# axruff/cuda-flow2d

Hardware: AMD Instinct MI355X
Metric: Mpixels*SOR-iters/sec at finest level (whole-pyramid wall time); full-pyramid pairs/sec in pairs_per_s (higher is better)
Workload: dtype f32; 1 GPU; cfg3_4096_gradient; width=4096, height=4096, pyramid_levels=8, data_constancy=gradient, median_radius=5, relaxation=Jacobi, reference iteration counts (bit-exact parity mode), parallelism=independent pairs, one process per GPU, no data-path collective, streams_per_gpu=4, hip_graph_replay=True, steps_per_lock_step_group=8

## Files before the change

cuda-flow2d_amd/__init__.py:

```python
import ctypes as C
import math
import os
import subprocess

import numpy as np

_HERE = os.path.dirname(os.path.abspath(__file__))
ROOT = os.path.dirname(_HERE)
HIP_LIB_PATH = os.environ.get("FLOW2D_HIP_LIB") or os.path.join(_HERE, "csrc", "libflow2d_hip.so")
HOST_LIB_PATH = os.path.join(_HERE, "host", "libflow2d_host.so")
CLI_PATH = os.path.join(_HERE, "host", "flow2d")

GREY, GRADIENT, GRADIENT_UNTILED, LOG_DERIVATIVES = 0, 1, 2, 3
_HOST_CONSTANCY = {GREY: 0, GRADIENT: 1, GRADIENT_UNTILED: 3, LOG_DERIVATIVES: 2}
SOLVER_AUTO, SOLVER_PER_SWEEP, SOLVER_FUSED, SOLVER_SINGLE_WORKGROUP, SOLVER_TILED = 0, 1, 2, 3, 4
TRACK_ALIVE, TRACK_INACTIVE, TRACK_MOTION_BOUNDARY, TRACK_LEFT_FRAME, TRACK_OCCLUDED = 0, 1, 2, 3, 4
DEFAULT_MIN_EIGENVALUE = 1.0
MOTION_TRANSLATION, MOTION_SIMILARITY, MOTION_AFFINE = 0, 1, 2
MOTION_MODELS = {"translation": MOTION_TRANSLATION, "similarity": MOTION_SIMILARITY, "affine": MOTION_AFFINE}

STATUS = {0: "ok", 1: "invalid argument", 2: "no usable HIP device", 3: "HIP runtime error",
          4: "out of device memory", 5: "unsupported parameter"}


# ... 181 lines not shown
        L.flow2d_context_destroy.argtypes = [vp]
        L.flow2d_context_device.argtypes = [vp, C.POINTER(i)]
        L.flow2d_context_stream.argtypes = [vp, C.POINTER(vp)]
        L.flow2d_synchronize.argtypes = [vp]
        L.flow2d_context_set_batch.argtypes = [vp, sz, sz]
        L.flow2d_mem_info.argtypes = [vp, C.POINTER(sz), C.POINTER(sz)]
        L.flow2d_device_name.argtypes = [vp, C.c_char_p, sz]
        L.flow2d_plane_pitch_bytes.restype = sz
        L.flow2d_plane_pitch_bytes.argtypes = [sz]
        L.flow2d_plane_alloc.argtypes = [vp, sz, sz, C.POINTER(vp), C.POINTER(sz)]
        L.flow2d_plane_free.argtypes = [vp, vp]
        L.flow2d_memset_2d.argtypes = [vp, vp, sz, i, sz, sz]
        L.flow2d_copy_h2d_2d.argtypes = [vp, vp, sz, vp, sz, sz, sz]
        L.flow2d_copy_d2h_2d.argtypes = [vp, vp, sz, vp, sz, sz, sz]
        L.flow2d_copy_d2d.argtypes = [vp, vp, vp, sz]
        L.flow2d_copy_planes.argtypes = [vp, sz, C.POINTER(vp), C.POINTER(vp), sz, sz, sz]
        L.flow2d_event_create.argtypes = [vp, C.POINTER(vp)]
        L.flow2d_event_record.argtypes = [vp, vp]
        L.flow2d_event_synchronize.argtypes = [vp, vp]
        L.flow2d_event_elapsed_ms.argtypes = [vp, vp, vp, C.POINTER(f)]
        L.flow2d_event_destroy.argtypes = [vp, vp]
        L.flow2d_stream_wait_event.argtypes = [vp, vp]
        L.flow2d_host_alloc.argtypes = [vp, sz, C.POINTER(vp)]
        L.flow2d_host_free.argtypes = [vp, vp]
        L.flow2d_add_2d.argtypes = [vp, vp, vp, sz, sz, sz]
        L.flow2d_gaussian_kernel.argtypes = [f, C.POINTER(f), C.POINTER(i)]
        L.flow2d_convolution_rows.argtypes = [vp, vp, vp, sz, sz, sz, C.POINTER(f), i]
        L.flow2d_convolution_columns.argtypes = [vp, vp, vp, sz, sz, sz, C.POINTER(f), i]
        L.flow2d_gaussian_blur.argtypes = [vp, vp, vp, sz, sz, sz, C.POINTER(f), i]
        L.flow2d_median_2d.argtypes = [vp, vp, sz, sz, sz, sz, vp]
        L.flow2d_registration_2d.argtypes = [vp, vp, vp, vp, vp, sz, sz, sz, f, f, vp]
        L.flow2d_upsample_registration_2d.argtypes = [vp, vp, vp, sz, sz, vp, vp, vp, vp, sz, sz, sz, f, f, vp]
        L.flow2d_resample_x.argtypes = [vp, vp, vp, sz, sz, sz, sz]
        L.flow2d_resample_y.argtypes = [vp, vp, vp, sz, sz, sz, sz]
        L.flow2d_add_2d_pair.argtypes = [vp, vp, vp, vp, vp, sz, sz, sz]
        L.flow2d_median_2d_pair.argtypes = [vp, vp, vp, sz, sz, sz, sz, vp, vp]
        L.flow2d_add_median_2d_pair.argtypes = [vp, vp, vp, vp, vp, sz, sz, sz, sz, vp, vp]
        L.flow2d_resample_x_pair.argtypes = [vp, vp, vp, vp, vp, sz, sz, sz, sz]
        L.flow2d_resample_y_pair.argtypes = [vp, vp, vp, vp, vp, sz, sz, sz, sz]
        L.flow2d_resample_xy_pair.argtypes = [vp, vp, vp, vp, vp, sz, sz, sz, sz, sz]
        L.flow2d_resample_x_levels.argtypes = [vp, vp, vp, vp, vp, sz, sz, sz, sz, C.POINTER(sz), C.POINTER(sz)]
        L.flow2d_compute_phi_ksi.argtypes = [vp] * 7 + [sz, sz, sz, f, f, f, f, vp, vp]
        L.flow2d_solve_2d.argtypes = [vp] * 9 + [sz, sz, sz, f, f, f, vp, vp]
        L.flow2d_solve_2d_grad.argtypes = [vp] * 9 + [sz, sz, sz, f, f, f, vp, vp]
        L.flow2d_solve_2d_grad_untiled.argtypes = [vp] * 9 + [sz, sz, sz, f, f, f, vp, vp]
        L.flow2d_solve_2d_log.argtypes = [vp] * 9 + [sz, sz, sz, f, f, f, vp, vp]
        L.flow2d_solver_algorithm_for.argtypes = [i, sz, sz, sz, sz, sz, i]
        L.flow2d_solve_2d_sor.argtypes = [vp] * 9 + [sz, sz, sz, f, f, f, f, i]
        L.flow2d_solve_level.argtypes = [vp] * 11 + [C.POINTER(SolveParams), C.POINTER(i)]
        L.flow2d_timing_enable.argtypes = [vp, i]
        L.flow2d_fused_fallbacks.argtypes = [vp, C.POINTER(C.c_ulonglong)]
        L.flow2d_context_set_lone.argtypes = [vp, i]
        L.flow2d_resample_y_levels.argtypes = [vp, vp, vp, vp, vp, sz, sz, sz, C.POINTER(sz), C.POINTER(sz), C.POINTER(sz), C.POINTER(sz)]
        L.flow2d_clock_probe_start.argtypes = [vp, C.c_double]
        L.flow2d_clock_probe_read.argtypes = [vp, C.POINTER(C.c_double)]
        L.flow2d_fused_block_order.argtypes = [vp, sz, sz, sz, sz, C.POINTER(i), sz, C.POINTER(sz)]
        if hasattr(L, "flow2d_fused_plain_waves"):
            L.flow2d_fused_plain_waves.argtypes = [vp, C.POINTER(C.c_ulonglong)]
        L.flow2d_timing_launch_filter.argtypes = [vp, sz, sz]
        if hasattr(L, "flow2d_consistency_2d"):
            L.flow2d_consistency_2d.argtypes = [vp, vp, vp, vp, vp, sz, sz, sz, f, f, vp]
        if hasattr(L, "flow2d_interpolate_2d"):
            L.flow2d_interpolate_2d.argtypes = [vp] * 9 + [sz, sz, sz, f, i, f, vp]
        if hasattr(L, "flow2d_track_points_2d"):
            L.flow2d_track_points_2d.argtypes = [vp] * 5 + [sz, sz, sz, vp, vp, vp, sz, f, f, i, f, f, vp, vp, vp]
            L.flow2d_seed_points_workspace_bytes.restype = sz
            L.flow2d_seed_points_workspace_bytes.argtypes = [sz, sz, sz]
            L.flow2d_seed_points_2d.argtypes = [vp, vp, sz, sz, sz, sz, f, vp, vp, vp, sz, vp, vp, sz]
        if hasattr(L, "flow2d_denoise_2d"):
            L.flow2d_denoise_2d.argtypes = [vp, vp, sz, C.POINTER(vp), C.POINTER(vp), C.POINTER(vp), C.POINTER(vp), sz, sz, sz, f,
                                            vp, vp]
            L.flow2d_compose_flow_2d.argtypes = [vp] * 7 + [sz, sz, sz, vp, vp, vp]
        if hasattr(L, "flow2d_global_motion_2d"):
            d = C.c_double
            L.flow2d_global_motion_workspace_bytes.restype = sz
            L.flow2d_global_motion_workspace_bytes.argtypes = [sz, sz, sz]
            L.flow2d_global_motion_2d.argtypes = [vp, vp, vp, vp, sz, sz, sz, i, d, i, vp, vp, sz]
            L.flow2d_global_flow_2d.argtypes = [vp, vp, vp, vp, vp, sz, sz, sz, d, vp, vp, vp, vp, vp]
            L.flow2d_warp_global_2d.argtypes = [vp, vp, vp, sz, sz, sz, f, vp, vp]
        if hasattr(L, "flow2d_deformation_2d"):
            L.flow2d_deformation_workspace_bytes.restype = sz
            L.flow2d_deformation_workspace_bytes.argtypes = [sz, sz, sz]
            L.flow2d_deformation_2d.argtypes = [vp, vp, vp, vp, sz, sz, sz, i, C.POINTER(DeformationPlanes), vp, vp, sz]
        if hasattr(L, "flow2d_segment_motion_2d"):
            L.flow2d_segment_motion_workspace_bytes.restype = sz
            L.flow2d_segment_motion_workspace_bytes.argtypes = [sz, sz, sz]
            L.flow2d_segment_motion_2d.argtypes = [vp, vp, vp, vp, sz, sz, sz, f, f, C.c_uint, vp, vp, sz, vp, vp, sz]
        if hasattr(L, "flow2d_flow_error_2d"):
            L.flow2d_flow_error_workspace_bytes.restype = sz
            L.flow2d_flow_error_workspace_bytes.argtypes = [sz, sz, sz]
            L.flow2d_flow_error_2d.argtypes = [vp] * 6 + [sz, sz, sz, vp, vp, vp, vp, sz]
        L.flow2d_timing_count.argtypes = [vp, C.POINTER(sz)]
        L.flow2d_timing_get.argtypes = [vp, sz, C.POINTER(TimingRecord)]
        L.flow2d_timing_reset.argtypes = [vp]
        _hip = L
    return _hip


def _check(status, where):
    if status != 0:
        raise Flow2DError(status, where, hip_lib().flow2d_last_error().decode(errors="replace"))


def device_count():
    n = C.c_int(0)
    st = hip_lib().flow2d_device_count(C.byref(n))
    return n.value if st == 0 else 0


def gaussian_kernel(sigma):
    taps = (C.c_float * 51)()
    r = C.c_int(0)
    _check(hip_lib().flow2d_gaussian_kernel(sigma, taps, C.byref(r)), "flow2d_gaussian_kernel")
    return np.array(taps[: 2 * r.value + 1], np.float32), r.value


class Plane:

    def __init__(self, ctx, width, height):
        self.ctx = ctx
        self.width, self.height = width, height
        ptr, pitch = C.c_void_p(), C.c_size_t()
        _check(hip_lib().flow2d_plane_alloc(ctx.handle, width, height, C.byref(ptr), C.byref(pitch)),
               "flow2d_plane_alloc")
        self.ptr, self.pitch = ptr.value, pitch.value

    def upload(self, array):
        a = np.ascontiguousarray(array, np.float32)
        h, w = a.shape
        assert w <= self.width and h <= self.height
        _check(hip_lib().flow2d_copy_h2d_2d(self.ctx.handle, self.ptr, self.pitch, a.ctypes.data, w * 4, w * 4, h),
               "flow2d_copy_h2d_2d")
        self.ctx.synchronize()
        return self

    def download(self, width=None, height=None):
        w = self.width if width is None else width
        h = self.height if height is None else height
        out = np.empty((h, w), np.float32)
        _check(hip_lib().flow2d_copy_d2h_2d(self.ctx.handle, out.ctypes.data, w * 4, self.ptr, self.pitch, w * 4, h),
               "flow2d_copy_d2h_2d")
        self.ctx.synchronize()
        return out

    def fill_bytes(self, value=0):
        _check(hip_lib().flow2d_memset_2d(self.ctx.handle, self.ptr, self.pitch, value, self.width * 4, self.height),
               "flow2d_memset_2d")
        return self

    def free(self):
        if self.ptr:
            hip_lib().flow2d_plane_free(self.ctx.handle, self.ptr)
            self.ptr = None


class _BatchScope:
# ... 9 lines not shown


class Context:

    def __init__(self, device=0, stream=None):
        h = C.c_void_p()
        if stream is None:
            _check(hip_lib().flow2d_context_create(device, C.byref(h)), "flow2d_context_create")
        else:
            _check(hip_lib().flow2d_context_create_on_stream(device, stream, C.byref(h)),
                   "flow2d_context_create_on_stream")
        self.handle = h
        self._planes = []

    def plane(self, width, height, data=None):
        p = Plane(self, width, height)
        self._planes.append(p)
        if data is not None:
            p.fill_bytes(0)
            p.upload(data)
        return p

    def copy_planes(self, srcs, dsts, width, height):
        n = len(srcs)
        a, b = (C.c_void_p * n)(*[p.ptr for p in srcs]), (C.c_void_p * n)(*[p.ptr for p in dsts])
        _check(hip_lib().flow2d_copy_planes(self.handle, n, a, b, srcs[0].pitch, width, height), "flow2d_copy_planes")

    def synchronize(self):
        _check(hip_lib().flow2d_synchronize(self.handle), "flow2d_synchronize")

    def mem_info(self):
        a, b = C.c_size_t(), C.c_size_t()
        _check(hip_lib().flow2d_mem_info(self.handle, C.byref(a), C.byref(b)), "flow2d_mem_info")
        return a.value, b.value

    def fused_fallbacks(self):
        n = C.c_ulonglong()
        _check(hip_lib().flow2d_fused_fallbacks(self.handle, C.byref(n)), "flow2d_fused_fallbacks")
        return n.value

    def set_lone(self, lone):
        _check(hip_lib().flow2d_context_set_lone(self.handle, int(bool(lone))), "flow2d_context_set_lone")

    def set_batch(self, count, stride_bytes=0):
        _check(hip_lib().flow2d_context_set_batch(self.handle, count, stride_bytes), "flow2d_context_set_batch")
        return _BatchScope(self)

    def resample_y_levels(self, packed_a, out_a, in_height, widths, heights, columns, rows, packed_b=None, out_b=None):
        n = len(widths)
        arr = lambda v: (C.c_size_t * n)(*v)
        _check(hip_lib().flow2d_resample_y_levels(self.handle, packed_a.ptr, out_a.ptr, packed_b.ptr if packed_b else None,
                                                  out_b.ptr if out_b else None, in_height, packed_a.pitch, n, arr(widths), arr(heights),
                                                  arr(columns), arr(rows)), "flow2d_resample_y_levels")

    def clock_probe_start(self, duration_us):
        _check(hip_lib().flow2d_clock_probe_start(self.handle, float(duration_us)), "flow2d_clock_probe_start")

    def clock_probe_read(self):
        ghz = (C.c_double * 8)()
        _check(hip_lib().flow2d_clock_probe_read(self.handle, ghz), "flow2d_clock_probe_read")
        return list(ghz)

    def fused_block_order(self, width, height, inner, instances=1):
        grid = C.c_size_t(0)
        cap = 1 << 16
        buf = (C.c_int * (4 * cap))()
        _check(hip_lib().flow2d_fused_block_order(self.handle, width, height, inner, instances, buf, cap, C.byref(grid)),
               "flow2d_fused_block_order")
        return np.frombuffer(buf, np.int32, 4 * grid.value).reshape(-1, 4).copy()

    def fused_plain_waves(self):
        n = C.c_ulonglong()
        _check(hip_lib().flow2d_fused_plain_waves(self.handle, C.byref(n)), "flow2d_fused_plain_waves")
        return n.value

    def device_name(self):
        buf = C.create_string_buffer(256)
        _check(hip_lib().flow2d_device_name(self.handle, buf, 256), "flow2d_device_name")
        return buf.value.decode()

    def close(self):
        if self.handle:
            for p in self._planes:
                p.free()
            self._planes = []
            hip_lib().flow2d_context_destroy(self.handle)
            self.handle = None

    def __enter__(self):
        return self

    def __exit__(self, *exc):
        self.close()

    def event(self):
        e = C.c_void_p()
        _check(hip_lib().flow2d_event_create(self.handle, C.byref(e)), "flow2d_event_create")
        return e

    def record(self, ev):
        _check(hip_lib().flow2d_event_record(self.handle, ev), "flow2d_event_record")

    def wait_event(self, ev):
        _check(hip_lib().flow2d_event_synchronize(self.handle, ev), "flow2d_event_synchronize")

    def elapsed_ms(self, start, stop):
# ... 967 lines not shown
```

cuda-flow2d_amd/csrc/pyramid_ops.hip:

```cpp
#include <algorithm>
#include <cmath>
#include <type_traits>
#include <utility>

#include "common.hpp"

namespace {

constexpr int kBlockX = 64;
constexpr int kBlockY = 4;

inline dim3 grid_for(size_t w, size_t h) { return dim3(flow2d::div_up(w, kBlockX), flow2d::div_up(h, kBlockY)); }

__global__ __launch_bounds__(256) void add_2d_kernel(float* __restrict__ op0_a, const float* __restrict__ op1_a,
                                                     float* __restrict__ op0_b, const float* __restrict__ op1_b, int w,
                                                     int h, int pitch, BatchArg batch)
{
    float* __restrict__ op0 = (batch_plane(batch) ? op0_b : op0_a) + batch_offset(batch);
    const float* __restrict__ op1 = (batch_plane(batch) ? op1_b : op1_a) + batch_offset(batch);
    const int x4 = (blockIdx.x * kBlockX + threadIdx.x) * 4;
    const int y = blockIdx.y * kBlockY + threadIdx.y;
    if (y >= h || x4 >= w) return;
    const size_t off = static_cast<size_t>(y) * pitch + x4;
    if (x4 + 3 < w) {
        float4 a = *reinterpret_cast<const float4*>(op0 + off);
        const float4 b = *reinterpret_cast<const float4*>(op1 + off);
        a.x += b.x;
        a.y += b.y;
        a.z += b.z;
        a.w += b.w;
        *reinterpret_cast<float4*>(op0 + off) = a;
    } else {
        for (int i = 0; x4 + i < w; ++i) op0[off + i] += op1[off + i];
    }
}

struct GaussTaps {
    float t[51];
};

template <bool kRows>
__global__ __launch_bounds__(256) void gauss_kernel(float* __restrict__ dst, const float* __restrict__ src, int w,
                                                    int h, int pitch, int radius, GaussTaps taps)
{
    const int x = blockIdx.x * kBlockX + threadIdx.x;
    const int y = blockIdx.y * kBlockY + threadIdx.y;
    if (x >= w || y >= h) return;
    float sum = 0.f;
    for (int j = -radius; j <= radius; ++j) {
        float s;
        if (kRows) {
            const int xx = x + j;
            s = (xx >= 0 && xx < w) ? src[static_cast<size_t>(y) * pitch + xx] : 0.f;
// ... 709 lines not shown
    const int out_w = lv.out_w[l], out_h = lv.out_h[l], rows_per_thread = lv.rows_per_thread[l];
    const float delta = lv.delta[l], normalization = lv.normalization[l];
    const float* __restrict__ in = (batch_plane(batch) ? in_b : in_a) + batch_offset(batch) + lv.col[l];
    float* __restrict__ out = (batch_plane(batch) ? out_b : out_a) + batch_offset(batch) + static_cast<size_t>(lv.out_row[l]) * pitch;
    const int block = static_cast<int>(blockIdx.x) - lv.first_block[l], blocks_x = lv.blocks_x[l];
    const int block_y = block / blocks_x;
    const int x = (block - block_y * blocks_x) * kBlockX + threadIdx.x;
    if (x >= out_w) return;
    const float* base = in + x;
    const int max_cells = lv.max_cells[l];
    if (rows_per_thread == 4 && max_cells <= 2) return resample_y_rows<2, 4>(base, out, x, block_y, out_h, in_h, pitch, delta, normalization);
    if (rows_per_thread == 4 && max_cells <= 4) return resample_y_rows<4, 4>(base, out, x, block_y, out_h, in_h, pitch, delta, normalization);
    if (rows_per_thread == 4 && max_cells <= 9) return resample_y_rows<9, 4>(base, out, x, block_y, out_h, in_h, pitch, delta, normalization);
    if (rows_per_thread == 1 && max_cells <= 9) return resample_y_rows<9, 1>(base, out, x, block_y, out_h, in_h, pitch, delta, normalization);
    for (int row = 0; row < rows_per_thread; ++row) {
        const int y = (block_y * rows_per_thread + row) * kBlockY + threadIdx.y;
        if (y >= out_h) return;
        const float left_f = static_cast<float>(static_cast<unsigned>(y)) * delta;
        const float right_f = static_cast<float>(static_cast<unsigned>(y) + 1u) * delta;
        const int left_i = static_cast<int>(floorf(left_f));
        const int right_i = min(in_h, static_cast<int>(ceilf(right_f)));
        const int cells = right_i - left_i;
        const size_t stride = pitch;
        float value = 0.f;
        if (cells == 1) {
            value += base[static_cast<size_t>(left_i) * stride] * delta;
        } else if (cells > 1) {
            const int last = left_i + cells - 1;
            value += base[static_cast<size_t>(left_i) * stride] * (static_cast<float>(left_i + 1) - left_f);
            int k = left_i + 1;
            for (; k + 32 <= last; k += 32) {
                float v[32];
#pragma unroll
                for (int i = 0; i < 32; ++i) v[i] = base[static_cast<size_t>(k + i) * stride];
#pragma unroll
                for (int i = 0; i < 32; ++i) value += v[i];
            }
            for (; k < last; k += 8) {
                float v[8];
#pragma unroll
                for (int i = 0; i < 8; ++i) v[i] = base[static_cast<size_t>(min(k + i, last - 1)) * stride];
#pragma unroll
                for (int i = 0; i < 8; ++i) {
                    const float next = value + v[i];
                    value = k + i < last ? next : value;
                }
            }
            value += base[static_cast<size_t>(last) * stride] * (right_f - static_cast<float>(last));
        }
        out[static_cast<size_t>(y) * pitch + x] = value * normalization;
    }
}

}

extern "C" {

static int launch_add(flow2d_context* ctx, float* operand_0, const float* operand_1, float* operand_0_b,
                      const float* operand_1_b, size_t width, size_t height, size_t pitch_bytes)
{
    FLOW2D_ENTER(ctx);
    if (!flow2d::plane_args_ok(operand_0, width, height, pitch_bytes) ||
        !flow2d::plane_args_ok(operand_1, width, height, pitch_bytes))
        return FLOW2D_ERR_INVALID_ARGUMENT;
    const bool pair = operand_0_b || operand_1_b;
    if (pair && (!flow2d::plane_args_ok(operand_0_b, width, height, pitch_bytes) ||
                 !flow2d::plane_args_ok(operand_1_b, width, height, pitch_bytes) || operand_0_b == operand_0 ||
                 operand_0_b == operand_1 || operand_0 == operand_1_b))
        return FLOW2D_ERR_INVALID_ARGUMENT;
    const unsigned planes = pair ? 2 : 1;
    dim3 grid(flow2d::div_up(width, kBlockX * 4), flow2d::div_up(height, kBlockY), flow2d::batch_z(ctx, planes));
    add_2d_kernel<<<grid, dim3(kBlockX, kBlockY), 0, ctx->stream>>>(operand_0, operand_1, operand_0_b, operand_1_b,
                                                                   (int)width, (int)height, (int)(pitch_bytes / 4),
                                                                   flow2d::batch_arg(ctx, planes));
    FLOW2D_CHECK_LAUNCH();
    return FLOW2D_OK;
}

int flow2d_add_2d(flow2d_context* ctx, float* operand_0, const float* operand_1, size_t width, size_t height,
                  size_t pitch_bytes)
{
    return launch_add(ctx, operand_0, operand_1, nullptr, nullptr, width, height, pitch_bytes);
}

int flow2d_add_2d_pair(flow2d_context* ctx, float* operand_0_a, const float* operand_1_a, float* operand_0_b,
                       const float* operand_1_b, size_t width, size_t height, size_t pitch_bytes)
{
    if (!operand_0_b || !operand_1_b) return FLOW2D_ERR_INVALID_ARGUMENT;
    return launch_add(ctx, operand_0_a, operand_1_a, operand_0_b, operand_1_b, width, height, pitch_bytes);
}

namespace {
struct PlaneTable {
    const float* src[FLOW2D_COPY_PLANES_MAX];
    float* dst[FLOW2D_COPY_PLANES_MAX];
};
__global__ __launch_bounds__(256) void copy_planes_kernel(PlaneTable t, int width, int height, int pitch_floats)
{
    const float* src = t.src[blockIdx.z];
    float* dst = t.dst[blockIdx.z];
    const int quads = width >> 2;
    for (int y = blockIdx.y; y < height; y += gridDim.y) {
        const size_t row = static_cast<size_t>(y) * pitch_floats;
        for (int q = blockIdx.x * blockDim.x + threadIdx.x; q < quads; q += gridDim.x * blockDim.x)
            reinterpret_cast<float4*>(dst + row)[q] = reinterpret_cast<const float4*>(src + row)[q];
        const int x = (quads << 2) + blockIdx.x * blockDim.x + threadIdx.x;
// ... 198 lines not shown
        }
    }
    const size_t lds_bytes = (in_width + in_width / 32 + 1) * sizeof(float);
    resample_x_levels_kernel<<<dim3(static_cast<unsigned>(height), 1, flow2d::batch_z(ctx, planes)), 256, lds_bytes,
                               ctx->stream>>>(input_a, packed_a, input_b, packed_b, static_cast<int>(in_width),
                                              static_cast<int>(pitch), lv, flow2d::batch_arg(ctx, planes));
    FLOW2D_CHECK_LAUNCH();
    return FLOW2D_OK;
}

int flow2d_resample_y_levels(flow2d_context* ctx, const float* packed_a, float* output_a, const float* packed_b, float* output_b,
                             size_t in_height, size_t pitch_bytes, size_t level_count, const size_t* out_widths,
                             const size_t* out_heights, const size_t* column_offsets, const size_t* output_rows)
{
    FLOW2D_ENTER(ctx);
    if (!out_widths || !out_heights || !column_offsets || !output_rows || level_count == 0 || !packed_a || !output_a ||
        packed_a == output_a || pitch_bytes == 0 || pitch_bytes % 16 != 0 || in_height == 0)
        return FLOW2D_ERR_INVALID_ARGUMENT;
    if (level_count > FLOW2D_RESAMPLE_MAX_LEVELS) return FLOW2D_ERR_UNSUPPORTED;
    const bool pair = packed_b || output_b;
    if (pair && (!packed_b || !output_b || packed_b == output_b || output_b == output_a || output_b == packed_a || output_a == packed_b))
        return FLOW2D_ERR_INVALID_ARGUMENT;
    const size_t pitch = pitch_bytes / 4;
    ResampleYLevels lv{};
    lv.count = static_cast<int>(level_count);
    long blocks = 0;
    for (size_t l = 0; l <= FLOW2D_RESAMPLE_MAX_LEVELS; ++l) lv.first_block[l] = 0x7fffffff;
    for (size_t l = 0; l < level_count; ++l) {
        if (out_widths[l] == 0 || out_heights[l] == 0 || out_heights[l] >= (1u << 30) || column_offsets[l] + out_widths[l] > pitch ||
            output_rows[l] >= (1u << 30))
            return FLOW2D_ERR_INVALID_ARGUMENT;
        for (size_t m = 0; m < l; ++m)
            if (output_rows[l] < output_rows[m] + out_heights[m] && output_rows[m] < output_rows[l] + out_heights[l])
                return FLOW2D_ERR_INVALID_ARGUMENT;
        lv.out_w[l] = static_cast<int>(out_widths[l]), lv.out_h[l] = static_cast<int>(out_heights[l]);
        lv.col[l] = static_cast<int>(column_offsets[l]), lv.out_row[l] = static_cast<int>(output_rows[l]);
        const float out_n = static_cast<float>(out_heights[l]), in_n = static_cast<float>(in_height);
        lv.delta[l] = in_n / out_n, lv.normalization[l] = out_n / in_n;
        lv.rows_per_thread[l] = out_widths[l] * out_heights[l] >= (size_t)512 * 512 ? 4 : 1;
        lv.max_cells[l] = lv.delta[l] == std::floor(lv.delta[l]) && lv.delta[l] < 1e6f ? static_cast<int>(lv.delta[l])
                                                                                      : static_cast<int>(std::min(std::ceil(lv.delta[l]) + 2.f, 1e9f));
        lv.first_block[l] = static_cast<int>(blocks);
        lv.blocks_x[l] = static_cast<int>(flow2d::div_up(out_widths[l], kBlockX));
        blocks += static_cast<long>(lv.blocks_x[l]) * static_cast<long>(flow2d::div_up(flow2d::div_up(out_heights[l], lv.rows_per_thread[l]), kBlockY));
        if (blocks >= 0x7fffffffl) return FLOW2D_ERR_UNSUPPORTED;
    }
    const unsigned planes = pair ? 2 : 1;
    resample_y_levels_kernel<<<dim3(static_cast<unsigned>(blocks), 1, flow2d::batch_z(ctx, planes)), dim3(kBlockX, kBlockY), 0, ctx->stream>>>(
        packed_a, output_a, packed_b, output_b, static_cast<int>(in_height), static_cast<int>(pitch), lv, flow2d::batch_arg(ctx, planes));
    FLOW2D_CHECK_LAUNCH();
    return FLOW2D_OK;
}

int flow2d_resample_x(flow2d_context* ctx, const float* input, float* output, size_t out_width, size_t out_height,
                      size_t in_width, size_t pitch_bytes)
{
    return launch_resample(ctx, true, input, output, nullptr, nullptr, out_width, out_height, in_width, pitch_bytes);
}

int flow2d_resample_x_pair(flow2d_context* ctx, const float* input_a, float* output_a, const float* input_b,
                           float* output_b, size_t out_width, size_t out_height, size_t in_width, size_t pitch_bytes)
{
    if (!input_b || !output_b) return FLOW2D_ERR_INVALID_ARGUMENT;
    return launch_resample(ctx, true, input_a, output_a, input_b, output_b, out_width, out_height, in_width, pitch_bytes);
}

int flow2d_resample_y(flow2d_context* ctx, const float* input, float* output, size_t out_width, size_t out_height,
                      size_t in_height, size_t pitch_bytes)
{
    return launch_resample(ctx, false, input, output, nullptr, nullptr, out_width, out_height, in_height, pitch_bytes);
}

int flow2d_resample_y_pair(flow2d_context* ctx, const float* input_a, float* output_a, const float* input_b,
                           float* output_b, size_t out_width, size_t out_height, size_t in_height, size_t pitch_bytes)
{
    if (!input_b || !output_b) return FLOW2D_ERR_INVALID_ARGUMENT;
    return launch_resample(ctx, false, input_a, output_a, input_b, output_b, out_width, out_height, in_height,
                           pitch_bytes);
}

int flow2d_resample_xy_pair(flow2d_context* ctx, const float* input_a, float* output_a, const float* input_b,
                            float* output_b, size_t in_width, size_t in_height, size_t out_width, size_t out_height,
                            size_t pitch_bytes)
{
    FLOW2D_ENTER(ctx);
    if (!flow2d::plane_args_ok(input_a, in_width, in_height, pitch_bytes) ||
        !flow2d::plane_args_ok(output_a, out_width, out_height, pitch_bytes) || input_a == output_a)
        return FLOW2D_ERR_INVALID_ARGUMENT;
    const bool pair = input_b || output_b;
    if (pair && (!flow2d::plane_args_ok(input_b, in_width, in_height, pitch_bytes) ||
                 !flow2d::plane_args_ok(output_b, out_width, out_height, pitch_bytes) || input_b == output_b ||
                 output_b == output_a || output_b == input_a || output_a == input_b))
        return FLOW2D_ERR_INVALID_ARGUMENT;
    const unsigned planes = pair ? 2 : 1;
    dim3 grid = grid_for(out_width, flow2d::div_up(out_height, kResampleXYRows));
    grid.z = flow2d::batch_z(ctx, planes);
    const ResampleXY k{static_cast<float>(in_width) / static_cast<float>(out_width),
                       static_cast<float>(out_width) / static_cast<float>(in_width),
                       static_cast<float>(in_height) / static_cast<float>(out_height),
                       static_cast<float>(out_height) / static_cast<float>(in_height)};
    resample_xy_kernel<<<grid, dim3(kBlockX, kBlockY), 0, ctx->stream>>>(
        input_a, output_a, input_b, output_b, (int)out_width, (int)out_height, (int)in_width, (int)in_height,
        (int)(pitch_bytes / 4), k, flow2d::batch_arg(ctx, planes));
    FLOW2D_CHECK_LAUNCH();
    return FLOW2D_OK;
}
// ... 66 lines not shown
```

cuda-flow2d_amd/host/optical_flow_2d.cpp:

```cpp
#include "optical_flow_2d.h"

#include <algorithm>
#include <cmath>
#include <cstdio>

#include "host_entry.h"

size_t OpticalFlowBase2D::GetMaxWarpLevel(size_t width, size_t height, float scale_factor) const
{
    size_t level_w = 1, level_h = 1, levels = 1;
    for (; scale_factor < 1.f; ++levels) {
        const float s = std::pow(scale_factor, static_cast<float>(levels));
        level_w = static_cast<size_t>(std::ceil(width * s));
        level_h = static_cast<size_t>(std::ceil(height * s));
        if (level_w < 4 || level_h < 4) break;
    }
    if (level_w == 1 || level_h == 1) --levels;
    return levels;
}

bool OpticalFlowBase2D::IsInitialized() const
{
    if (!initialized_) std::printf("Error: '%s' was not initialized.\n", name_);
    return initialized_;
// ... 677 lines not shown
        DevicePtr temp = Acquire();
        for (int i = 0; i < 2; ++i) {
            FramePyramid& pyramid = *sequence_frames_[i];
            if (gaussian_sigma > 0.0) {
                pyramid.level0 = pyramid.blurred;
                if (!pyramid.valid) {
                    op.Clear();
                    op.PushValuePtr("dev_input", &callers[i]);
                    op.PushValuePtr("dev_output", &pyramid.level0);
                    op.PushValuePtr("dev_temp", &temp);
                    op.PushValuePtr("data_size", &original_size);
                    op.PushValuePtr("gaussian_sigma", &gaussian_sigma);
                    cuop_convolution_.Execute(op);
                failed |= cuop_convolution_.TakeFailure();
                }
            } else {
                pyramid.level0 = callers[i];
            }
            *level0[i] = pyramid.level0;
        }
        Release(temp);
    } else if (gaussian_sigma > 0.0 && caller_frame_0_) {
        DevicePtr temp = Acquire();
        DevicePtr sources[2] = {caller_frame_0_, caller_frame_1_};
        DevicePtr* targets[2] = {&frame_0, &frame_1};
        for (int i = 0; i < 2; ++i) {
            op.Clear();
            op.PushValuePtr("dev_input", &sources[i]);
            op.PushValuePtr("dev_output", targets[i]);
            op.PushValuePtr("dev_temp", &temp);
            op.PushValuePtr("data_size", &original_size);
            op.PushValuePtr("gaussian_sigma", &gaussian_sigma);
            cuop_convolution_.Execute(op);
            failed |= cuop_convolution_.TakeFailure();
        }
        Release(temp);
    } else if (gaussian_sigma > 0.0) {
        DevicePtr temp = Acquire();
        DevicePtr* io[2][2] = {{&frame_0, &flow_u}, {&frame_1, &flow_v}};
        for (auto& pair : io) {
            op.Clear();
            op.PushValuePtr("dev_input", pair[0]);
            op.PushValuePtr("dev_output", pair[1]);
            op.PushValuePtr("dev_temp", &temp);
            op.PushValuePtr("data_size", &original_size);
            op.PushValuePtr("gaussian_sigma", &gaussian_sigma);
            cuop_convolution_.Execute(op);
            failed |= cuop_convolution_.TakeFailure();
            std::swap(*pair[0], *pair[1]);
        }
        Release(temp);
    }

    if (packed) {
        if (CheckFlow2DError(flow2d_resample_x_levels(context_, AsPlane(frame_0), AsPlane(packed_frames_[0]),
                                                      AsPlane(frame_1), AsPlane(packed_frames_[1]),
                                                      original_size.width, original_size.height,
                                                      dev_container_size_.pitch, packed_width.size(),
                                                      packed_width.data(), packed_column.data()),
                             "flow2d_resample_x_levels"))
            failed = true;
        if (stacked) {
            std::vector<size_t> widths, heights, rows;
            for (int l = first_level; l >= 1; --l) {
                widths.push_back(level_width[static_cast<size_t>(l)]);
                heights.push_back(level_height[static_cast<size_t>(l)]);
                rows.push_back(level_row[static_cast<size_t>(l)]);
            }
            if (CheckFlow2DError(flow2d_resample_y_levels(context_, AsPlane(packed_frames_[0]), AsPlane(frame_0_res), AsPlane(packed_frames_[1]),
                                                          AsPlane(frame_1_res), original_size.height, dev_container_size_.pitch, widths.size(),
                                                          widths.data(), heights.data(), packed_column.data(), rows.data()),
                                 "flow2d_resample_y_levels"))
                failed = true;
        }
    }

    DataSize3 current_size = {0, 0, 0}, prev_size = {0, 0, 0};
    for (; level >= 0; --level) {
        const float scale = std::pow(warp_scale_factor, static_cast<float>(level));
        current_size.width = static_cast<size_t>(std::ceil(original_size.width * scale));
        current_size.height = static_cast<size_t>(std::ceil(original_size.height * scale));
        float hx = original_size.width / static_cast<float>(current_size.width);
        float hy = original_size.height / static_cast<float>(current_size.height);
        if (!silent) std::printf("Solve level %2d (%4zu x%4zu) \n", level, current_size.width, current_size.height);

        DevicePtr sequence_level[2] = {frame_0, frame_1};
        if (sequence) {
            DevicePtr temp = level > 0 ? Acquire() : 0;
            for (int i = 0; i < 2 && level > 0; ++i) {
                FramePyramid& pyramid = *sequence_frames_[i];
                DevicePtr plane = SequenceLevelPlane(pyramid, static_cast<size_t>(level), current_size.height);
                if (!plane) {
                    Release(temp);
                    Release(frame_0_res);
                    Release(frame_1_res);
                    Release(flow_du);
                    Release(flow_dv);
                    return false;
                }
                if (!pyramid.valid) {
                    op.Clear();
                    op.PushValuePtr("dev_input", i == 0 ? &frame_0 : &frame_1);
                    op.PushValuePtr("dev_output", &plane);
                    op.PushValuePtr("dev_temp", &temp);
                    op.PushValuePtr("data_size", &original_size);
                    op.PushValuePtr("resample_size", &current_size);
                    cuop_resample_.Execute(op);
                failed |= cuop_resample_.TakeFailure();
                }
                sequence_level[i] = plane;
            }
            if (temp) Release(temp);
        } else if (stacked) {
        } else if (level == 0) {
            std::swap(frame_0, frame_0_res);
            std::swap(frame_1, frame_1_res);
        } else if (packed) {
            const size_t column = packed_column[static_cast<size_t>(first_level - level)];
            if (CheckFlow2DError(flow2d_resample_y_pair(context_, AsPlane(packed_frames_[0]) + column, AsPlane(frame_0_res),
                                                        AsPlane(packed_frames_[1]) + column, AsPlane(frame_1_res),
                                                        current_size.width, current_size.height, original_size.height,
                                                        dev_container_size_.pitch),
                                 "flow2d_resample_y_pair"))
                failed = true;
        } else {
            DevicePtr temp = Acquire(), temp_b = Acquire();
            op.Clear();
// ... 125 lines not shown
```

include/flow2d_c_abi.h:

```cpp
#ifndef FLOW2D_C_ABI_H_
#define FLOW2D_C_ABI_H_

#include <stddef.h>

#ifdef __cplusplus
extern "C" {
#endif

#define FLOW2D_API __attribute__((visibility("default")))

#define FLOW2D_ABI_VERSION 1

typedef enum flow2d_status {
    FLOW2D_OK = 0,
    FLOW2D_ERR_INVALID_ARGUMENT = 1,
    FLOW2D_ERR_NO_DEVICE = 2,
    FLOW2D_ERR_DEVICE = 3,
    FLOW2D_ERR_OUT_OF_MEMORY = 4,
    FLOW2D_ERR_UNSUPPORTED = 5
} flow2d_status;

typedef enum flow2d_constancy {
    FLOW2D_CONSTANCY_GREY = 0,
    FLOW2D_CONSTANCY_GRADIENT = 1,
// ... 251 lines not shown
#ifdef __cplusplus
static_assert(sizeof(flow2d_deformation_stats) == FLOW2D_DEFORMATION_STATS_BYTES, "flow2d_deformation_stats layout");
#else
_Static_assert(sizeof(flow2d_deformation_stats) == FLOW2D_DEFORMATION_STATS_BYTES, "flow2d_deformation_stats layout");
#endif

FLOW2D_API size_t flow2d_deformation_workspace_bytes(size_t width, size_t height, size_t instances);
FLOW2D_API int flow2d_deformation_2d(flow2d_context* ctx, const float* flow_u, const float* flow_v,
                                     const float* mask , size_t width, size_t height, size_t pitch_bytes,
                                     int measure, const flow2d_deformation_planes* out ,
                                     flow2d_deformation_stats* stats , void* workspace,
                                     size_t workspace_bytes);

FLOW2D_API int flow2d_upsample_registration_2d(flow2d_context* ctx, const float* flow_u, const float* flow_v, size_t in_width,
                                               size_t in_height, float* out_u, float* out_v, const float* frame_0,
                                               const float* frame_1, size_t width, size_t height, size_t pitch_bytes, float hx,
                                               float hy, float* output);

FLOW2D_API int flow2d_resample_x(flow2d_context* ctx, const float* input, float* output, size_t out_width,
                                 size_t out_height, size_t in_width, size_t pitch_bytes);
FLOW2D_API int flow2d_resample_y(flow2d_context* ctx, const float* input, float* output, size_t out_width,
                                 size_t out_height, size_t in_height, size_t pitch_bytes);

FLOW2D_API int flow2d_add_2d_pair(flow2d_context* ctx, float* operand_0_a, const float* operand_1_a,
                                  float* operand_0_b, const float* operand_1_b, size_t width, size_t height,
                                  size_t pitch_bytes);
FLOW2D_API int flow2d_median_2d_pair(flow2d_context* ctx, const float* input_a, const float* input_b, size_t width,
                                     size_t height, size_t pitch_bytes, size_t window, float* output_a,
                                     float* output_b);
FLOW2D_API int flow2d_add_median_2d_pair(flow2d_context* ctx, const float* input_a, const float* addend_a,
                                         const float* input_b, const float* addend_b, size_t width, size_t height,
                                         size_t pitch_bytes, size_t window, float* output_a, float* output_b);
FLOW2D_API int flow2d_resample_x_pair(flow2d_context* ctx, const float* input_a, float* output_a,
                                      const float* input_b, float* output_b, size_t out_width, size_t out_height,
                                      size_t in_width, size_t pitch_bytes);
FLOW2D_API int flow2d_resample_y_pair(flow2d_context* ctx, const float* input_a, float* output_a,
                                      const float* input_b, float* output_b, size_t out_width, size_t out_height,
                                      size_t in_height, size_t pitch_bytes);

FLOW2D_API int flow2d_resample_xy_pair(flow2d_context* ctx, const float* input_a, float* output_a, const float* input_b,
                                       float* output_b, size_t in_width, size_t in_height, size_t out_width,
                                       size_t out_height, size_t pitch_bytes);

#define FLOW2D_RESAMPLE_MAX_LEVELS 16
FLOW2D_API int flow2d_resample_x_levels(flow2d_context* ctx, const float* input_a, float* packed_a, const float* input_b,
                                        float* packed_b, size_t in_width, size_t height, size_t pitch_bytes,
                                        size_t level_count, const size_t* out_widths, const size_t* column_offsets);

FLOW2D_API int flow2d_resample_y_levels(flow2d_context* ctx, const float* packed_a, float* output_a, const float* packed_b,
                                        float* output_b, size_t in_height, size_t pitch_bytes, size_t level_count,
                                        const size_t* out_widths, const size_t* out_heights, const size_t* column_offsets,
                                        const size_t* output_rows);

FLOW2D_API int flow2d_compute_phi_ksi(flow2d_context* ctx, const float* frame_0, const float* frame_1,
                                      const float* flow_u, const float* flow_v, const float* flow_du,
                                      const float* flow_dv, size_t width, size_t height, size_t pitch_bytes, float hx,
                                      float hy, float equation_smoothness, float equation_data, float* phi,
                                      float* ksi);

FLOW2D_API int flow2d_solve_2d(flow2d_context* ctx, const float* frame_0, const float* frame_1, const float* flow_u,
                               const float* flow_v, const float* flow_du, const float* flow_dv, const float* phi,
                               const float* ksi, size_t width, size_t height, size_t pitch_bytes, float hx, float hy,
                               float equation_alpha, float* temp_du, float* temp_dv);

FLOW2D_API int flow2d_solve_2d_grad_untiled(flow2d_context* ctx, const float* frame_0, const float* frame_1,
                                            const float* flow_u, const float* flow_v, const float* flow_du,
                                            const float* flow_dv, const float* phi, const float* ksi, size_t width,
                                            size_t height, size_t pitch_bytes, float hx, float hy,
                                            float equation_alpha, float* temp_du, float* temp_dv);

FLOW2D_API int flow2d_solve_2d_grad(flow2d_context* ctx, const float* frame_0, const float* frame_1,
                                    const float* flow_u, const float* flow_v, const float* flow_du,
                                    const float* flow_dv, const float* phi, const float* ksi, size_t width,
                                    size_t height, size_t pitch_bytes, float hx, float hy, float equation_alpha,
                                    float* temp_du, float* temp_dv);

FLOW2D_API int flow2d_solve_2d_log(flow2d_context* ctx, const float* frame_0, const float* frame_1,
                                   const float* flow_u, const float* flow_v, const float* flow_du,
                                   const float* flow_dv, const float* phi, const float* ksi, size_t width,
                                   size_t height, size_t pitch_bytes, float hx, float hy, float equation_alpha,
                                   float* temp_du, float* temp_dv);

FLOW2D_API int flow2d_solve_2d_sor(flow2d_context* ctx, const float* frame_0, const float* frame_1,
                                   const float* flow_u, const float* flow_v, float* flow_du, float* flow_dv,
                                   const float* phi, const float* ksi, size_t width, size_t height, size_t pitch_bytes,
                                   float hx, float hy, float equation_alpha, float omega, int data_constancy);

typedef enum flow2d_solver_algorithm {
    FLOW2D_SOLVER_AUTO = 0,
    FLOW2D_SOLVER_PER_SWEEP = 1,
    FLOW2D_SOLVER_FUSED = 2,
    FLOW2D_SOLVER_SINGLE_WORKGROUP = 3,
    FLOW2D_SOLVER_TILED = 4
} flow2d_solver_algorithm;

typedef struct flow2d_solve_params {
    size_t width, height;
    size_t pitch_bytes;
    size_t container_height;
    float hx, hy;
    float equation_alpha;
    float equation_smoothness;
    float equation_data;
    size_t outer_iterations_count;
    size_t inner_iterations_count;
    int data_constancy;
// ... 43 lines not shown
```

Baseline: 305,000 Mpixel*iters/s.

## Fuse x and y pyramid resampling of all levels into one kernel

```diff
diff --git a/cuda-flow2d_amd/__init__.py b/cuda-flow2d_amd/__init__.py
--- a/cuda-flow2d_amd/__init__.py
+++ b/cuda-flow2d_amd/__init__.py
@@ -257,6 +257,9 @@
         L.flow2d_fused_fallbacks.argtypes = [vp, C.POINTER(C.c_ulonglong)]
         L.flow2d_context_set_lone.argtypes = [vp, i]
         L.flow2d_resample_y_levels.argtypes = [vp, vp, vp, vp, vp, sz, sz, sz, C.POINTER(sz), C.POINTER(sz), C.POINTER(sz), C.POINTER(sz)]
+        L.flow2d_resample_xy_levels.argtypes = [vp, vp, vp, vp, vp, sz, sz, sz, sz, C.POINTER(sz), C.POINTER(sz), C.POINTER(sz), C.POINTER(sz)]
+        L.flow2d_resample_xy_levels_launches.argtypes = []
+        L.flow2d_resample_xy_levels_launches.restype = C.c_ulonglong
         L.flow2d_clock_probe_start.argtypes = [vp, C.c_double]
         L.flow2d_clock_probe_read.argtypes = [vp, C.POINTER(C.c_double)]
         L.flow2d_fused_block_order.argtypes = [vp, sz, sz, sz, sz, C.POINTER(i), sz, C.POINTER(sz)]
@@ -307,6 +310,10 @@
         raise Flow2DError(status, where, hip_lib().flow2d_last_error().decode(errors="replace"))
 
 
+def resample_xy_levels_launches():
+    return int(hip_lib().flow2d_resample_xy_levels_launches())
+
+
 def device_count():
     n = C.c_int(0)
     st = hip_lib().flow2d_device_count(C.byref(n))
@@ -422,6 +429,15 @@
         _check(hip_lib().flow2d_resample_y_levels(self.handle, packed_a.ptr, out_a.ptr, packed_b.ptr if packed_b else None,
                                                   out_b.ptr if out_b else None, in_height, packed_a.pitch, n, arr(widths), arr(heights),
                                                   arr(columns), arr(rows)), "flow2d_resample_y_levels")
+
+    def resample_xy_levels(self, src_a, out_a, in_width, in_height, widths, heights, rows, columns=None, src_b=None, out_b=None,
+                           pitch=None):
+        n = len(widths)
+        arr = lambda v: (C.c_size_t * n)(*v)
+        ptr = lambda p: None if p is None else (p if isinstance(p, int) else p.ptr)
+        _check(hip_lib().flow2d_resample_xy_levels(self.handle, ptr(src_a), ptr(out_a), ptr(src_b), ptr(out_b), in_width, in_height,
+                                                   src_a.pitch if pitch is None else pitch, n, arr(widths), arr(heights), arr(rows),
+                                                   arr(columns) if columns is not None else None), "flow2d_resample_xy_levels")
 
     def clock_probe_start(self, duration_us):
         _check(hip_lib().flow2d_clock_probe_start(self.handle, float(duration_us)), "flow2d_clock_probe_start")
diff --git a/cuda-flow2d_amd/csrc/pyramid_ops.hip b/cuda-flow2d_amd/csrc/pyramid_ops.hip
--- a/cuda-flow2d_amd/csrc/pyramid_ops.hip
+++ b/cuda-flow2d_amd/csrc/pyramid_ops.hip
@@ -1,4 +1,5 @@
 #include <algorithm>
+#include <atomic>
 #include <cmath>
 #include <type_traits>
 #include <utility>
@@ -814,6 +815,227 @@
     }
 }
 
+constexpr int kXYCells = 16;
+constexpr int kXYRows = 16;
+constexpr int kXYWaveCols = 64 * kXYCells;
+constexpr int kXYMaxLog = 8;
+constexpr int kXYDeepLog = 5;
+constexpr int kXYStageWords = kXYWaveCols + 4 * (kXYWaveCols / 32 + kXYWaveCols / 256) + 8;
+
+struct ResampleXYLevels {
+    unsigned present;
+    int col[kXYMaxLog + 1], row[kXYMaxLog + 1];
+};
+
+__device__ __forceinline__ float xy_norm(int k) { return __int_as_float((127 - k) << 23); }
+
+__device__ __forceinline__ void xy_wave_sync()
+{
+    __builtin_amdgcn_fence(__ATOMIC_RELEASE, "wavefront");
+    __builtin_amdgcn_wave_barrier();
+    __builtin_amdgcn_fence(__ATOMIC_ACQUIRE, "wavefront");
+}
+
+__device__ __forceinline__ int xy_deep_slot(int k) { return 64 - (64 >> (k - kXYDeepLog)); }
+
+template <int MAX_THREADS>
+__global__ __launch_bounds__(MAX_THREADS) void resample_xy_levels_kernel(const float* __restrict__ in_a, float* __restrict__ out_a,
+                                                                         const float* __restrict__ in_b, float* __restrict__ out_b,
+                                                                         int in_w, int in_h, int pitch, int band_rows, int col_ranges,
+                                                                         ResampleXYLevels lv, BatchArg batch)
+{
+    extern __shared__ float xy_lds[];
+    const float* __restrict__ in = (batch_plane(batch) ? in_b : in_a) + batch_offset(batch);
+    float* __restrict__ out = (batch_plane(batch) ? out_b : out_a) + batch_offset(batch);
+    const int lane = static_cast<int>(threadIdx.x) & 63, wave = static_cast<int>(threadIdx.x) >> 6;
+    const int waves = static_cast<int>(blockDim.x) >> 6;
+    const int band = static_cast<int>(blockIdx.x) / col_ranges;
+    const int c0 = (static_cast<int>(blockIdx.x) - band * col_ranges) * kXYWaveCols;
+    const unsigned present = lv.present;
+    const bool deep = (present >> kXYDeepLog) != 0;
+    float* __restrict__ stage = xy_lds + wave * kXYStageWords;
+    float* __restrict__ table = xy_lds + waves * kXYStageWords;
+
+    const int x = c0 + lane * kXYCells;
+    const bool active = x < in_w;
+    const int y0 = band * band_rows + wave * kXYRows;
+    const int rows = min(kXYRows, in_h - y0);
+    const float* __restrict__ src = in + static_cast<size_t>(y0) * pitch + x;
+
+    int deep_k = 0, deep_g = 0;
+    if (lane < 32) deep_k = 5, deep_g = lane;
+    else if (lane < 48) deep_k = 6, deep_g = lane - 32;
+    else if (lane < 56) deep_k = 7, deep_g = lane - 48;
+    else if (lane < 60) deep_k = 8, deep_g = lane - 56;
+    const bool chain = deep_k != 0 && ((present >> deep_k) & 1u) != 0 && c0 + ((deep_g + 1) << deep_k) <= in_w;
+
+    float acc1[8], acc2[4], acc3[2], acc4 = 0.f;
+#pragma unroll
+    for (int o = 0; o < 8; ++o) acc1[o] = 0.f;
+#pragma unroll
+    for (int o = 0; o < 4; ++o) acc2[o] = 0.f;
+    acc3[0] = acc3[1] = 0.f;
+
+    float4 buf[4][kXYCells / 4];
+    auto load = [&](float4 (&dst)[kXYCells / 4], int r) {
+        const float4* __restrict__ p = reinterpret_cast<const float4*>(src + static_cast<size_t>(r) * pitch);
+#pragma unroll
+        for (int q = 0; q < kXYCells / 4; ++q) dst[q] = p[q];
+    };
+    auto process = [&](const float4 (&cells)[kXYCells / 4], int r) {
+        const int y = y0 + r;
+        if (active) {
+            float c[kXYCells];
+#pragma unroll
+            for (int q = 0; q < kXYCells / 4; ++q) c[4 * q] = cells[q].x, c[4 * q + 1] = cells[q].y, c[4 * q + 2] = cells[q].z, c[4 * q + 3] = cells[q].w;
+            if (deep) {
+                float4* __restrict__ mine = reinterpret_cast<float4*>(stage + pow2_lds_index(lane * kXYCells));
+#pragma unroll
+                for (int q = 0; q < kXYCells / 4; ++q) mine[q] = cells[q];
+            }
+            float s2[8], s4[4], s8[2], s16;
+#pragma unroll
+            for (int o = 0; o < 8; ++o) s2[o] = (0.f + c[2 * o]) + c[2 * o + 1];
+#pragma unroll
+            for (int o = 0; o < 4; ++o) s4[o] = (s2[2 * o] + c[4 * o + 2]) + c[4 * o + 3];
+#pragma unroll
+            for (int o = 0; o < 2; ++o) s8[o] = (((s4[2 * o] + c[8 * o + 4]) + c[8 * o + 5]) + c[8 * o + 6]) + c[8 * o + 7];
+            s16 = s8[0];
+#pragma unroll
+            for (int j = 8; j < 16; ++j) s16 += c[j];
+            if (present & 2u) {
+#pragma unroll
+                for (int o = 0; o < 8; ++o) acc1[o] += s2[o] * 0.5f;
+                if ((r & 1) == 1) {
+                    float4* __restrict__ dst = reinterpret_cast<float4*>(out + static_cast<size_t>(lv.row[1] + (y >> 1)) * pitch + lv.col[1] + (x >> 1));
+                    dst[0] = make_float4(acc1[0] * 0.5f, acc1[1] * 0.5f, acc1[2] * 0.5f, acc1[3] * 0.5f);
+                    dst[1] = make_float4(acc1[4] * 0.5f, acc1[5] * 0.5f, acc1[6] * 0.5f, acc1[7] * 0.5f);
+#pragma unroll
+                    for (int o = 0; o < 8; ++o) acc1[o] = 0.f;
+                }
+            }
+            if (present & 4u) {
+#pragma unroll
+                for (int o = 0; o < 4; ++o) acc2[o] += s4[o] * 0.25f;
+                if ((r & 3) == 3) {
+                    *reinterpret_cast<float4*>(out + static_cast<size_t>(lv.row[2] + (y >> 2)) * pitch + lv.col[2] + (x >> 2)) =
+                        make_float4(acc2[0] * 0.25f, acc2[1] * 0.25f, acc2[2] * 0.25f, acc2[3] * 0.25f);
+#pragma unroll
+                    for (int o = 0; o < 4; ++o) acc2[o] = 0.f;
+                }
+            }
+            if (present & 8u) {
+                acc3[0] += s8[0] * 0.125f, acc3[1] += s8[1] * 0.125f;
+                if ((r & 7) == 7) {
+                    *reinterpret_cast<float2*>(out + static_cast<size_t>(lv.row[3] + (y >> 3)) * pitch + lv.col[3] + (x >> 3)) =
+                        make_float2(acc3[0] * 0.125f, acc3[1] * 0.125f);
+                    acc3[0] = acc3[1] = 0.f;
+                }
+            }
+            if (present & 16u) {
+                acc4 += s16 * 0.0625f;
+                if ((r & 15) == 15) {
+                    out[static_cast<size_t>(lv.row[4] + (y >> 4)) * pitch + lv.col[4] + (x >> 4)] = acc4 * 0.0625f;
+                    acc4 = 0.f;
+                }
+            }
+        }
+        if (!deep) return;
+        xy_wave_sync();
+        if (chain) {
+            const int blocks = (1 << deep_k) / kXYCells;
+            const float* __restrict__ first = stage;
+            const int cell0 = deep_g << deep_k;
+            float value = 0.f;
+            auto read = [&](float4 (&dst)[kXYCells / 4], int b) {
+                const float4* __restrict__ block = reinterpret_cast<const float4*>(first + pow2_lds_index(cell0 + b * kXYCells));
+#pragma unroll
+                for (int q = 0; q < kXYCells / 4; ++q) dst[q] = block[q];
+            };
+            auto add = [&](const float4 (&v)[kXYCells / 4]) {
+#pragma unroll
+                for (int q = 0; q < kXYCells / 4; ++q) {
+                    value += v[q].x;
+                    value += v[q].y;
+                    value += v[q].z;
+                    value += v[q].w;
+                }
+            };
+            float4 a[kXYCells / 4], n[kXYCells / 4];
+            read(a, 0);
+            for (int b = 0; b < blocks; b += 2) {
+                read(n, b + 1);
+                __builtin_amdgcn_sched_barrier(0);
+                add(a);
+                __builtin_amdgcn_sched_barrier(0);
+                read(a, min(b + 2, blocks - 1));
+                __builtin_amdgcn_sched_barrier(0);
+                add(n);
+                __builtin_amdgcn_sched_barrier(0);
+            }
+            table[(wave * kXYRows + r) * 64 + lane] = value * xy_norm(deep_k);
+        }
+        xy_wave_sync();
+    };
+
+    if (active) {
+#pragma unroll
+        for (int p = 0; p < 3; ++p)
+            if (p < rows) load(buf[p], p);
+    }
+    for (int r0 = 0; r0 < rows; r0 += 4) {
+#pragma unroll
+        for (int u = 0; u < 4; ++u) {
+            const int r = r0 + u;
+            if (r < rows) {
+                if (active && r + 3 < rows) load(buf[(u + 3) & 3], r + 3);
+                __builtin_amdgcn_sched_barrier(0);
+                process(buf[u], r);
+            }
+        }
+    }
+    if (!deep) return;
+    __syncthreads();
+    int item = static_cast<int>(threadIdx.x);
+#pragma unroll
+    for (int k = kXYDeepLog; k <= kXYMaxLog; ++k) {
+        if (((present >> k) & 1u) == 0 || item < 0) continue;
+        const int per_row = kXYWaveCols >> k, count = per_row * (band_rows >> k);
+        if (item >= count) {
+            item -= count;
+            continue;
+        }
+        const int j = item / per_row, gl = item - j * per_row;
+        item = -1;
+        if (c0 + ((gl + 1) << k) > in_w) continue;
+        const float* __restrict__ column = table + (j << k) * 64 + xy_deep_slot(k) + gl;
+        float value = 0.f;
+        for (int rr = 0; rr < (1 << k); rr += 16) {
+            float v[16];
+#pragma unroll
+            for (int i = 0; i < 16; ++i) v[i] = column[(rr + i) * 64];
+#pragma unroll
+            for (int i = 0; i < 16; ++i) value += v[i];
+        }
+        out[static_cast<size_t>(lv.row[k] + band * (band_rows >> k) + j) * pitch + lv.col[k] + (c0 >> k) + gl] = value * xy_norm(k);
+    }
+}
+
+std::atomic<unsigned long long> xy_levels_launches{0};
+
+template <int MAX_THREADS>
+hipError_t xy_levels_allow_lds(int device)
+{
+    static std::atomic<unsigned long long> allowed{0};
+    const bool tracked = device >= 0 && device < 64;
+    if (tracked && ((allowed.load() >> device) & 1ull)) return hipSuccess;
+    constexpr int kBytes = ((MAX_THREADS / 64) * kXYStageWords + (MAX_THREADS / 4) * 64) * static_cast<int>(sizeof(float));
+    const hipError_t e = hipFuncSetAttribute(reinterpret_cast<const void*>(&resample_xy_levels_kernel<MAX_THREADS>),
+                                             hipFuncAttributeMaxDynamicSharedMemorySize, kBytes);
+    if (e == hipSuccess && tracked) allowed.fetch_or(1ull << device);
+    return e;
+}
+
 }
 
 extern "C" {
@@ -1118,6 +1340,88 @@
     return FLOW2D_OK;
 }
 
+int flow2d_resample_xy_levels(flow2d_context* ctx, const float* input_a, float* output_a, const float* input_b, float* output_b,
+                              size_t in_width, size_t in_height, size_t pitch_bytes, size_t level_count, const size_t* out_widths,
+                              const size_t* out_heights, const size_t* output_rows, const size_t* output_columns)
+{
+    FLOW2D_ENTER(ctx);
+    if (!out_widths || !out_heights || !output_rows || level_count == 0) return FLOW2D_ERR_INVALID_ARGUMENT;
+    const bool pair = input_b || output_b;
+    if (!flow2d::plane_args_ok(input_a, in_width, in_height, pitch_bytes) || !output_a || (reinterpret_cast<uintptr_t>(output_a) % 16) != 0)
+        return FLOW2D_ERR_INVALID_ARGUMENT;
+    if (pair && (!flow2d::plane_args_ok(input_b, in_width, in_height, pitch_bytes) || !output_b || (reinterpret_cast<uintptr_t>(output_b) % 16) != 0))
+        return FLOW2D_ERR_INVALID_ARGUMENT;
+    if (level_count > FLOW2D_RESAMPLE_MAX_LEVELS || in_width % kPow2Cells != 0 || in_width > 256 * kPow2Cells) return FLOW2D_ERR_UNSUPPORTED;
+    const size_t pitch = pitch_bytes / 4;
+    ResampleXYLevels lv{};
+    int level_of[kXYMaxLog + 1];
+    for (int& l : level_of) l = -1;
+    int deepest = 0;
+    for (size_t l = 0; l < level_count; ++l) {
+        if (out_widths[l] == 0 || out_heights[l] == 0) return FLOW2D_ERR_INVALID_ARGUMENT;
+        const size_t ratio = in_width / out_widths[l];
+        if (ratio < 2 || ratio > (1u << kXYMaxLog) || (ratio & (ratio - 1)) != 0 || ratio * out_widths[l] != in_width ||
+            ratio * out_heights[l] != in_height)
+            return FLOW2D_ERR_UNSUPPORTED;
+        int k = 0;
+        while ((size_t{1} << k) < ratio) ++k;
+        if (level_of[k] >= 0) return FLOW2D_ERR_UNSUPPORTED;
+        level_of[k] = static_cast<int>(l);
+        deepest = std::max(deepest, k);
+    }
+    size_t first_row = ~size_t{0}, end_row = 0;
+    for (size_t l = 0; l < level_count; ++l) {
+        const size_t column = output_columns ? output_columns[l] : 0;
+        if (column % 4 != 0 || column + out_widths[l] > pitch || output_rows[l] >= (1u << 30)) return FLOW2D_ERR_INVALID_ARGUMENT;
+        for (size_t m = 0; m < l; ++m) {
+            const size_t column_m = output_columns ? output_columns[m] : 0;
+            const bool rows_meet = output_rows[l] < output_rows[m] + out_heights[m] && output_rows[m] < output_rows[l] + out_heights[l];
+            const bool columns_meet = column < column_m + out_widths[m] && column_m < column + out_widths[l];
+            if (rows_meet && columns_meet) return FLOW2D_ERR_INVALID_ARGUMENT;
+        }
+        first_row = std::min(first_row, output_rows[l]);
+        end_row = std::max(end_row, output_rows[l] + out_heights[l]);
+    }
+    {
+        const size_t written_span = flow2d::batch_span(ctx, (end_row - first_row) * pitch_bytes);
+        const size_t read_span = flow2d::batch_span(ctx, in_height * pitch_bytes);
+        const flow2d::ByteRange written[] = {{output_a + first_row * pitch, written_span}, {pair ? output_b + first_row * pitch : nullptr, written_span}};
+        const flow2d::ByteRange read[] = {{input_a, read_span}, {input_b, read_span}};
+        if (flow2d::any_overlap(written, read)) return FLOW2D_ERR_INVALID_ARGUMENT;
+    }
+    for (int k = 1; k <= kXYMaxLog; ++k) {
+        if (level_of[k] < 0) continue;
+        lv.present |= 1u << k;
+        lv.col[k] = static_cast<int>(output_columns ? output_columns[level_of[k]] : 0);
+        lv.row[k] = static_cast<int>(output_rows[level_of[k]]);
+    }
+    const bool deep = deepest >= kXYDeepLog;
+    const int band_rows = deep ? 1 << deepest : kXYRows;
+    const int waves = band_rows / kXYRows;
+    const unsigned col_ranges = flow2d::div_up(in_width, kXYWaveCols);
+    const size_t blocks = static_cast<size_t>(col_ranges) * flow2d::div_up(in_height, band_rows);
+    if (blocks >= 0x7fffffffull) return FLOW2D_ERR_UNSUPPORTED;
+    const size_t lds_bytes = deep ? (static_cast<size_t>(waves) * kXYStageWords + static_cast<size_t>(band_rows) * 64) * sizeof(float) : 0;
+    const unsigned planes = pair ? 2 : 1;
+    const dim3 grid(static_cast<unsigned>(blocks), 1, flow2d::batch_z(ctx, planes));
+    if (waves <= 8) {
+        FLOW2D_HIP_TRY(xy_levels_allow_lds<512>(ctx->device));
+        resample_xy_levels_kernel<512><<<grid, 64 * waves, lds_bytes, ctx->stream>>>(
+            input_a, output_a, input_b, output_b, static_cast<int>(in_width), static_cast<int>(in_height), static_cast<int>(pitch), band_rows,
+            static_cast<int>(col_ranges), lv, flow2d::batch_arg(ctx, planes));
+    } else {
+        FLOW2D_HIP_TRY(xy_levels_allow_lds<1024>(ctx->device));
+        resample_xy_levels_kernel<1024><<<grid, 64 * waves, lds_bytes, ctx->stream>>>(
+            input_a, output_a, input_b, output_b, static_cast<int>(in_width), static_cast<int>(in_height), static_cast<int>(pitch), band_rows,
+            static_cast<int>(col_ranges), lv, flow2d::batch_arg(ctx, planes));
+    }
+    FLOW2D_CHECK_LAUNCH();
+    xy_levels_launches.fetch_add(1, std::memory_order_relaxed);
+    return FLOW2D_OK;
+}
+
+unsigned long long flow2d_resample_xy_levels_launches(void) { return xy_levels_launches.load(std::memory_order_relaxed); }
+
 int flow2d_resample_x(flow2d_context* ctx, const float* input, float* output, size_t out_width, size_t out_height,
                       size_t in_width, size_t pitch_bytes)
 {
diff --git a/cuda-flow2d_amd/host/optical_flow_2d.cpp b/cuda-flow2d_amd/host/optical_flow_2d.cpp
--- a/cuda-flow2d_amd/host/optical_flow_2d.cpp
+++ b/cuda-flow2d_amd/host/optical_flow_2d.cpp
@@ -753,7 +753,24 @@
         Release(temp);
     }
 
-    if (packed) {
+    std::vector<size_t> widths, heights, rows;
+    if (stacked) {
+        for (int l = first_level; l >= 1; --l) {
+            widths.push_back(level_width[static_cast<size_t>(l)]);
+            heights.push_back(level_height[static_cast<size_t>(l)]);
+            rows.push_back(level_row[static_cast<size_t>(l)]);
+        }
+    }
+    bool fused_levels = false;
+    if (stacked) {
+        const int status = flow2d_resample_xy_levels(context_, AsPlane(frame_0), AsPlane(frame_0_res), AsPlane(frame_1), AsPlane(frame_1_res),
+                                                     original_size.width, original_size.height, dev_container_size_.pitch,
+                                                     widths.size(), widths.data(), heights.data(), rows.data(), nullptr);
+        fused_levels = status != FLOW2D_ERR_UNSUPPORTED && status != FLOW2D_ERR_INVALID_ARGUMENT;
+        if (fused_levels && CheckFlow2DError(status, "flow2d_resample_xy_levels")) failed = true;
+    }
+
+    if (packed && !fused_levels) {
         if (CheckFlow2DError(flow2d_resample_x_levels(context_, AsPlane(frame_0), AsPlane(packed_frames_[0]),
                                                       AsPlane(frame_1), AsPlane(packed_frames_[1]),
                                                       original_size.width, original_size.height,
@@ -761,19 +778,12 @@
                                                       packed_width.data(), packed_column.data()),
                              "flow2d_resample_x_levels"))
             failed = true;
-        if (stacked) {
-            std::vector<size_t> widths, heights, rows;
-            for (int l = first_level; l >= 1; --l) {
-                widths.push_back(level_width[static_cast<size_t>(l)]);
-                heights.push_back(level_height[static_cast<size_t>(l)]);
-                rows.push_back(level_row[static_cast<size_t>(l)]);
-            }
-            if (CheckFlow2DError(flow2d_resample_y_levels(context_, AsPlane(packed_frames_[0]), AsPlane(frame_0_res), AsPlane(packed_frames_[1]),
-                                                          AsPlane(frame_1_res), original_size.height, dev_container_size_.pitch, widths.size(),
-                                                          widths.data(), heights.data(), packed_column.data(), rows.data()),
-                                 "flow2d_resample_y_levels"))
-                failed = true;
-        }
+        if (stacked &&
+            CheckFlow2DError(flow2d_resample_y_levels(context_, AsPlane(packed_frames_[0]), AsPlane(frame_0_res), AsPlane(packed_frames_[1]),
+                                                      AsPlane(frame_1_res), original_size.height, dev_container_size_.pitch, widths.size(),
+                                                      widths.data(), heights.data(), packed_column.data(), rows.data()),
+                             "flow2d_resample_y_levels"))
+            failed = true;
     }
 
     DataSize3 current_size = {0, 0, 0}, prev_size = {0, 0, 0};
diff --git a/include/flow2d_c_abi.h b/include/flow2d_c_abi.h
--- a/include/flow2d_c_abi.h
+++ b/include/flow2d_c_abi.h
@@ -327,6 +327,12 @@
                                         const size_t* out_widths, const size_t* out_heights, const size_t* column_offsets,
                                         const size_t* output_rows);
 
+FLOW2D_API int flow2d_resample_xy_levels(flow2d_context* ctx, const float* input_a, float* output_a, const float* input_b,
+                                         float* output_b, size_t in_width, size_t in_height, size_t pitch_bytes, size_t level_count,
+                                         const size_t* out_widths, const size_t* out_heights, const size_t* output_rows,
+                                         const size_t* output_columns);
+FLOW2D_API unsigned long long flow2d_resample_xy_levels_launches(void);
+
 FLOW2D_API int flow2d_compute_phi_ksi(flow2d_context* ctx, const float* frame_0, const float* frame_1,
                                       const float* flow_u, const float* flow_v, const float* flow_du,
                                       const float* flow_dv, size_t width, size_t height, size_t pitch_bytes, float hx,
```

Measured after the change: 309,300 Mpixel*iters/s (median of 6 runs). 1.4% higher.
